# Copojacaab/APDA-FFT

Hardware: NVIDIA B200
Metric: FFT+peak windows/sec at N=4096 (higher is better)
Workload: dtype f32

## Files before the change

### apda-fft_b200/csrc/fft_f32_fast.cuh

```cuda
#pragma once
#include "common.cuh"

namespace {

__device__ __forceinline__ unsigned long long &u64(float2 &v) { return reinterpret_cast<unsigned long long &>(v); }
__device__ __forceinline__ const unsigned long long &u64(const float2 &v) {
    return reinterpret_cast<const unsigned long long &>(v);
}
__device__ __forceinline__ float2 cadd(float2 a, float2 b) {
    float2 r;
    asm("add.rn.f32x2 %0, %1, %2;" : "=l"(u64(r)) : "l"(u64(a)), "l"(u64(b)));
    return r;
}
__device__ __forceinline__ float2 csub(float2 a, float2 b) {
    float2 r;
    asm("sub.rn.f32x2 %0, %1, %2;" : "=l"(u64(r)) : "l"(u64(a)), "l"(u64(b)));
    return r;
}
__device__ __forceinline__ float2 pmul(float2 a, float2 b) {
    float2 r;
    asm("mul.rn.f32x2 %0, %1, %2;" : "=l"(u64(r)) : "l"(u64(a)), "l"(u64(b)));
    return r;
}
__device__ __forceinline__ float2 pfma(float2 a, float2 b, float2 c) {
    float2 r;
    asm("fma.rn.f32x2 %0, %1, %2, %3;" : "=l"(u64(r)) : "l"(u64(a)), "l"(u64(b)), "l"(u64(c)));
    return r;
}
__device__ __forceinline__ float2 cmul(float2 a, float2 w) {
    return make_float2(fmaf(a.x, w.x, -a.y * w.y), fmaf(a.x, w.y, a.y * w.x));
}

#define SQRT1_2f 0.70710678118654752440f
#define COS_PI_8f 0.92387953251128675613f
#define SIN_PI_8f 0.38268343236508977173f

__device__ __forceinline__ void add_sub_mi(float2 u, float2 d, float2 &plus, float2 &minus) {
    plus = make_float2(u.x + d.y, u.y - d.x);
    minus = make_float2(u.x - d.y, u.y + d.x);
}

__device__ __forceinline__ void fft4(float2 &a0, float2 &a1, float2 &a2, float2 &a3) {
    const float2 t0 = cadd(a0, a2), t1 = csub(a0, a2), t2 = cadd(a1, a3), d = csub(a1, a3);
    a0 = cadd(t0, t2);
    a2 = csub(t0, t2);
    add_sub_mi(t1, d, a1, a3);
}
__device__ __forceinline__ void fft8(float2 *v) {
    float2 e0 = v[0], e1 = v[2], e2 = v[4], e3 = v[6];
    float2 o0 = v[1], o1 = v[3], o2 = v[5], o3 = v[7];
    fft4(e0, e1, e2, e3);
    fft4(o0, o1, o2, o3);
    o1 = pmul(make_float2(o1.x + o1.y, o1.y - o1.x), make_float2(SQRT1_2f, SQRT1_2f));
    o3 = pmul(make_float2(o3.y - o3.x, o3.x + o3.y), make_float2(SQRT1_2f, -SQRT1_2f));
    v[0] = cadd(e0, o0);
    v[4] = csub(e0, o0);
    v[1] = cadd(e1, o1);
    v[5] = csub(e1, o1);
    add_sub_mi(e2, o2, v[2], v[6]);
    v[3] = cadd(e3, o3);
    v[7] = csub(e3, o3);
}
__device__ __forceinline__ void fft16(float2 *v) {
    float2 e[8], o[8];
#pragma unroll
    for (int i = 0; i < 8; ++i) {
        e[i] = v[2 * i];
        o[i] = v[2 * i + 1];
    }
    fft8(e);
    fft8(o);
    const float2 w1 = make_float2(COS_PI_8f, -SIN_PI_8f), w3 = make_float2(SIN_PI_8f, -COS_PI_8f);
    const float2 w5 = make_float2(-SIN_PI_8f, -COS_PI_8f), w7 = make_float2(-COS_PI_8f, -SIN_PI_8f);
    o[1] = cmul(o[1], w1);
    o[2] = pmul(make_float2(o[2].x + o[2].y, o[2].y - o[2].x), make_float2(SQRT1_2f, SQRT1_2f));
    o[3] = cmul(o[3], w3);
    o[5] = cmul(o[5], w5);
    o[6] = pmul(make_float2(o[6].y - o[6].x, o[6].x + o[6].y), make_float2(SQRT1_2f, -SQRT1_2f));
    o[7] = cmul(o[7], w7);
#pragma unroll
    for (int i = 0; i < 8; ++i) {
        if (i == 4) {
            add_sub_mi(e[4], o[4], v[4], v[12]);
        } else {
            v[i] = cadd(e[i], o[i]);
            v[i + 8] = csub(e[i], o[i]);
        }
    }
}
template <int R>
__device__ __forceinline__ void fft_r(float2 *v) {
    if (R == 16) fft16(v);
    else if (R == 8) fft8(v);
    else fft4(v[0], v[1], v[2], v[3]);
}

__constant__ float2 c_tw2_1024[64];
__constant__ float2 c_tw2_2048[64];
__constant__ float2 c_tw2_4096[128];
__constant__ float2 c_tw2_8192[256];
template <int N>
__device__ __forceinline__ const float2 *const_tw2() {
    return N == 1024 ? c_tw2_1024 : N == 2048 ? c_tw2_2048 : N == 4096 ? c_tw2_4096 : c_tw2_8192;
}

#ifndef APDA_K1_MINB_2048
#define APDA_K1_MINB_2048 8
#endif
#ifndef APDA_K1_MINB_1024
#define APDA_K1_MINB_1024 8
#endif
#ifndef APDA_K1_MINB_8192
#define APDA_K1_MINB_8192 4
#endif
#ifndef APDA_K1_MINB
#define APDA_K1_MINB 9
#endif
template <int N>
struct Plan;
template <>
struct Plan<8192> { static constexpr int R1 = 16, R2 = 16, R3 = 16, WPB = 1, MINB = APDA_K1_MINB_8192; };
template <>
struct Plan<4096> { static constexpr int R1 = 16, R2 = 16, R3 = 8, WPB = 1, MINB = APDA_K1_MINB; };
template <>
struct Plan<2048> { static constexpr int R1 = 16, R2 = 8, R3 = 8, WPB = 2, MINB = APDA_K1_MINB_2048; };
template <>
struct Plan<1024> { static constexpr int R1 = 8, R2 = 8, R3 = 8, WPB = 4, MINB = APDA_K1_MINB_1024; };

template <int T>
__device__ __forceinline__ void group_sync(int slot) {
    if (T == 32) __syncwarp();
    else if (slot == 0) asm volatile("bar.sync 1, %0;" ::"n"(T) : "memory");
    else asm volatile("bar.sync 2, %0;" ::"n"(T) : "memory");
}

__device__ __forceinline__ float next_above(float v) {
    float n = key_value(ordered_key(v) + 1u, 0.f);
    if (!(n > v)) n = key_value(ordered_key(v) + 2u, 0.f);
    return n;
}

__device__ __noinline__ float2 bracket_minmax(float2 a0, float2 a1, float2 a2, float2 a3, float2 a4, float2 a5, float2 a6,
                                              float2 a7, float2 a8, float2 a9, float2 a10, float2 a11, float2 a12, float2 a13,
                                              float2 a14, float2 a15, unsigned inb) {
    const float2 a[16] = {a0, a1, a2, a3, a4, a5, a6, a7, a8, a9, a10, a11, a12, a13, a14, a15};
    float vmin = CUDART_INF_F, vmax = -CUDART_INF_F;
#pragma unroll
    for (int i = 0; i < 16; ++i) {
        if (inb & (0x80000000u >> (2 * i))) {
            vmin = fminf(vmin, a[i].x);
            vmax = fmaxf(vmax, a[i].x);
        }
        if (inb & (0x80000000u >> (2 * i + 1))) {
            vmin = fminf(vmin, a[i].y);
            vmax = fmaxf(vmax, a[i].y);
        }
    }
#pragma unroll
    for (int o = 16; o > 0; o >>= 1) {
        vmin = fminf(vmin, __shfl_xor_sync(0xffffffffu, vmin, o));
        vmax = fmaxf(vmax, __shfl_xor_sync(0xffffffffu, vmax, o));
    }
    return make_float2(vmin, vmax);
}

constexpr int kTightenFrom = 4;
template <int T, bool FULL, typename Reload>
__device__ float select_median(const float2 (&v2)[16], int n_valid, uint32_t *sh , int t, int slot,
                               Reload reload ) {
#define VAL(i) (((i) & 1) ? v2[(i) >> 1].y : v2[(i) >> 1].x)
    constexpr int NW = (T + 31) / 32;
    const int lane = t & 31, warp = t >> 5;
    const int r_lo = (n_valid - 1) >> 1, r_hi = n_valid >> 1;
    float *shf = reinterpret_cast<float *>(sh);

    {
        float s1 = 0.f, s2 = 0.f;
        int cntv = 0;
#pragma unroll
        for (int c = 0; c < 16; c += 4) {
#pragma unroll
            for (int h = 0; h < 2; ++h) {
                const float raw = h ? v2[c].y : v2[c].x;
                const bool ok = FULL || raw < CUDART_INF_F;
                const float x = ok ? raw : 0.f;
                s1 += x;
                s2 = fmaf(x, x, s2);
                cntv += ok;
            }
        }
#pragma unroll
        for (int o = 16; o > 0; o >>= 1) {
            s1 += __shfl_xor_sync(0xffffffffu, s1, o);
            s2 += __shfl_xor_sync(0xffffffffu, s2, o);
        }
        if (!FULL) cntv = __reduce_add_sync(0xffffffffu, cntv);
        if (lane == 0) {
            shf[warp] = s1;
            shf[8 + warp] = s2;
            if (!FULL) sh[16 + warp] = (uint32_t)cntv;
        }
        if (t == 0) sh[48] = 0;
    }
    group_sync<T>(slot);
    float mean, sd;
    {
        float s1 = 0.f, s2 = 0.f;
        int cntv = FULL ? 8 * T : 0;
#pragma unroll
        for (int w = 0; w < NW; ++w) {
            s1 += shf[w];
            s2 += shf[8 + w];
            if (!FULL) cntv += (int)sh[16 + w];
        }
        const float inv = rcp_approx((float)max(cntv, 1));
        mean = s1 * inv;
        sd = sqrt_approx(fmaxf(fmaf(-mean, mean, s2 * inv), 0.f));
    }
    const float inv_density = fmaxf(2.5f * sd, 1e-30f) * rcp_approx((float)n_valid);

    float lo = -CUDART_INF_F, hi = CUDART_INF_F;
    int c_lo = 0, c_hi = n_valid;
    unsigned mask_lo = 0u, mask_hi = 0xffffffffu;
    if (!FULL) {
        mask_hi = 0u;
#pragma unroll
        for (int i = 0; i < 32; ++i) mask_hi = (mask_hi << 1) | (VAL(i) < CUDART_INF_F ? 1u : 0u);
    }
    float pivot = mean;
    for (int round = 0;; ++round) {
        if (round > 0) {
            if (c_hi - c_lo <= 32) break;
            if (round >= kTightenFrom) {
                const float2 mm = bracket_minmax(v2[0], v2[1], v2[2], v2[3], v2[4], v2[5], v2[6], v2[7], v2[8], v2[9], v2[10],
                                                 v2[11], v2[12], v2[13], v2[14], v2[15], ~mask_lo & mask_hi);
                if (lane == 0) {
                    shf[warp] = mm.x;
                    shf[8 + warp] = mm.y;
                }
                group_sync<T>(slot);
                float vmin = shf[0], vmax = shf[8];
#pragma unroll
                for (int w = 1; w < NW; ++w) {
                    vmin = fminf(vmin, shf[w]);
                    vmax = fmaxf(vmax, shf[8 + w]);
                }
                if (vmin == vmax) {
                    group_sync<T>(slot);
                    return vmin;
                }
                lo = vmin;
                hi = next_above(vmax);
            }
            const float lo_next = lo > -CUDART_INF_F ? next_above(lo) : -3.4028234e38f;
            if (!(lo_next < hi)) break;
            const float want = (float)r_lo + 0.5f;
            if (lo == -CUDART_INF_F) {
                pivot = hi - 1.5f * fmaxf((float)c_hi - want, 1.f) * inv_density * (float)(1 << min(round - 1, 20));
            } else if (hi == CUDART_INF_F) {
                pivot = lo + 1.5f * fmaxf(want - (float)c_lo, 1.f) * inv_density * (float)(1 << min(round - 1, 20));
            } else if (round % 3 == 2) {
                const uint32_t a = ordered_key(lo), b = ordered_key(hi);
                pivot = key_value(a + ((b - a) >> 1), 0.f);
            } else {
                pivot = lo + (hi - lo) * __fdividef(want - (float)c_lo, (float)(c_hi - c_lo));
            }
            if (!(pivot > lo)) pivot = lo_next;
            if (!(pivot < hi)) pivot = lo_next;
        }
        unsigned signs = 0;
        const float2 pv = make_float2(pivot, pivot);
#pragma unroll
        for (int i = 0; i < 16; ++i) {
            const float2 d = csub(v2[i], pv);
            signs = __funnelshift_l(__float_as_uint(d.x), signs, 1);
            signs = __funnelshift_l(__float_as_uint(d.y), signs, 1);
        }
        int cnt = __popc(signs);
        cnt = __reduce_add_sync(0xffffffffu, cnt);
        uint32_t *cslot = sh + 32 + 8 * (round & 1);
        if (lane == 0) cslot[warp] = (uint32_t)cnt;
        group_sync<T>(slot);
        int tot = 0;
#pragma unroll
        for (int w = 0; w < NW; ++w) tot += (int)cslot[w];
        if (tot <= r_lo) {
            lo = pivot;
            c_lo = tot;
            mask_lo = signs;
        } else if (tot > r_hi) {
            hi = pivot;
            c_hi = tot;
            mask_hi = signs;
        } else {
            float below = -CUDART_INF_F, above = CUDART_INF_F;
#pragma unroll
            for (int i = 0; i < 32; ++i) {
                if (VAL(i) < pivot) below = fmaxf(below, VAL(i));
                else above = fminf(above, VAL(i));
            }
#pragma unroll
            for (int o = 16; o > 0; o >>= 1) {
                below = fmaxf(below, __shfl_xor_sync(0xffffffffu, below, o));
                above = fminf(above, __shfl_xor_sync(0xffffffffu, above, o));
            }
            if (lane == 0) {
                shf[warp] = below;
                shf[8 + warp] = above;
            }
            group_sync<T>(slot);
#pragma unroll
            for (int w = 0; w < NW; ++w) {
                below = fmaxf(below, shf[w]);
                above = fminf(above, shf[8 + w]);
            }
            group_sync<T>(slot);
            return (below + above) * 0.5f;
        }
    }
    if (c_hi - c_lo > 32) {
        group_sync<T>(slot);
        return lo;
    }
    for (unsigned inb = ~mask_lo & mask_hi; inb; ) {
        const int q = __clz(inb);
        inb &= ~(0x80000000u >> q);
        const uint32_t pos = atomicAdd(&sh[48], 1u);
        if (pos < 32u) shf[pos] = reload(q);
    }
    group_sync<T>(slot);
    const int cnt = (int)sh[48];
    if (warp == 0) {
        float med;
        if (cnt > 32) {
            med = lo;
        } else {
            const float mine = lane < cnt ? shf[lane] : CUDART_INF_F;
            int rank = 0;
            for (int j = 0; j < cnt; ++j) {
                const float other = shf[j];
                rank += (other < mine) || (other == mine && j < lane);
            }
            const uint32_t m_lo = __ballot_sync(0xffffffffu, lane < cnt && rank == r_lo - c_lo);
            const uint32_t m_hi = __ballot_sync(0xffffffffu, lane < cnt && rank == r_hi - c_lo);
            const float a = __shfl_sync(0xffffffffu, mine, __ffs(m_lo) - 1);
            const float b = __shfl_sync(0xffffffffu, mine, __ffs(m_hi) - 1);
            med = (a + b) * 0.5f;
        }
        if (lane == 0) shf[49] = med;
    }
    group_sync<T>(slot);
    return shf[49];
}
#undef VAL

template <int N, int CENTER, bool FULL, int PF_AHEAD = 0>
__device__ __forceinline__ void k1_forward(const float *__restrict__ samples, const int n_samples, const int64_t ld,
                                           const int64_t winc, const float2 *__restrict__ tw1, float2 *s, uint32_t *sel_w,
                                           float *red_w, const int wslot, const int t, const int64_t pf_batch = 0) {
    constexpr int center = CENTER;
    using P = Plan<N>;
    constexpr int M = N / 2, R1 = P::R1, R2 = P::R2, R3 = P::R3, T = M / 16;
    constexpr int S1 = R2 * R3;
    constexpr int LD = S1 + 16 / R1;
    constexpr int G1 = 16 / R1, G2 = 16 / R2, G3 = 16 / R3;
    float2 v[16];
    const float *x = samples + winc * ld;
    const float2 *z = reinterpret_cast<const float2 *>(x);
    const bool full = FULL;
#pragma unroll
    for (int g = 0; g < G1; ++g) {
        const int c = t + T * g;
#pragma unroll
        for (int n1 = 0; n1 < R1; ++n1) {
            const int zi = n1 * S1 + c;
            float2 val;
            if (FULL) {
                val = __ldg(z + zi);
            } else {
                val.x = (2 * zi < n_samples) ? __ldg(x + 2 * zi) : 0.f;
                val.y = (2 * zi + 1 < n_samples) ? __ldg(x + 2 * zi + 1) : 0.f;
            }
            v[g * R1 + n1] = val;
        }
    }
    if (APDA_L2_PREFETCH && PF_AHEAD > 0) {
        const int64_t wn = winc + (int64_t)sm_count_reg() * PF_AHEAD;
        if (wn < pf_batch) l2_prefetch_span(samples + wn * ld, n_samples * (int)sizeof(float), t, T);
    }
    float shift = 0.f;
    if (center == APDA_CENTER_MEDIAN) {
        if (!full) {
#pragma unroll
            for (int g = 0; g < G1; ++g)
#pragma unroll
                for (int n1 = 0; n1 < R1; ++n1) {
                    const int zi = n1 * S1 + t + T * g;
                    if (2 * zi >= n_samples) v[g * R1 + n1].x = CUDART_INF_F;
                    if (2 * zi + 1 >= n_samples) v[g * R1 + n1].y = CUDART_INF_F;
                }
        }
        auto reload = [&](int q) {
            const int j = q >> 1;
            return __ldg(x + 2 * ((j % R1) * S1 + t + T * (j / R1)) + (q & 1));
        };
        shift = select_median<T, FULL>(v, n_samples, sel_w, t, wslot, reload);
        if (!full) {
#pragma unroll
            for (int i = 0; i < 16; ++i) {
                if (v[i].x == CUDART_INF_F) v[i].x = 0.f;
                if (v[i].y == CUDART_INF_F) v[i].y = 0.f;
            }
        }
    } else if (center == APDA_CENTER_MEAN) {
        float acc = 0.f;
#pragma unroll
        for (int i = 0; i < 16; ++i) acc += v[i].x + v[i].y;
#pragma unroll
        for (int o = 16; o > 0; o >>= 1) acc += __shfl_xor_sync(0xffffffffu, acc, o);
        if ((t & 31) == 0) red_w[t >> 5] = acc;
        group_sync<T>(wslot);
        float tot = 0.f;
#pragma unroll
        for (int w = 0; w < (T + 31) / 32; ++w) tot += red_w[w];
        shift = tot / (float)n_samples;
    }
#pragma unroll
    for (int g = 0; g < G1; ++g) {
        const int c = t + T * g;
        if (center != APDA_CENTER_NONE) {
#pragma unroll
            for (int n1 = 0; n1 < R1; ++n1) {
                const int zi = n1 * S1 + c;
                if (full) {
                    v[g * R1 + n1] = csub(v[g * R1 + n1], make_float2(shift, shift));
                } else {
                    if (2 * zi < n_samples) v[g * R1 + n1].x -= shift;
                    if (2 * zi + 1 < n_samples) v[g * R1 + n1].y -= shift;
                }
            }
        }
        fft_r<R1>(v + g * R1);
        s[c] = v[g * R1];
#pragma unroll
        for (int k1 = 1; k1 < R1; ++k1) s[k1 * LD + c] = cmul(v[g * R1 + k1], __ldg(tw1 + k1 * S1 + c));
    }
    group_sync<T>(wslot);

    const float2 *tw2 = const_tw2<N>();
#pragma unroll
    for (int g = 0; g < G2; ++g) {
        const int w = t + T * g;
        const int k1 = w % R1, n3 = w / R1;
        float2 *col = s + k1 * LD + n3;
#pragma unroll
        for (int n2 = 0; n2 < R2; ++n2) v[g * R2 + n2] = col[n2 * R3];
        fft_r<R2>(v + g * R2);
        col[0] = v[g * R2];
#pragma unroll
        for (int k2 = 1; k2 < R2; ++k2) col[k2 * R3] = cmul(v[g * R2 + k2], tw2[k2 * R3 + n3]);
    }
    group_sync<T>(wslot);

#pragma unroll
    for (int g = 0; g < G3; ++g) {
        const int w = t + T * g;
        const int k1 = w % R1, k2 = w / R1;
        const float2 *row = s + k1 * LD + k2 * R3;
#pragma unroll
        for (int n3 = 0; n3 < R3; ++n3) v[g * R3 + n3] = row[n3];
        fft_r<R3>(v + g * R3);
    }
    group_sync<T>(wslot);
#pragma unroll
    for (int g = 0; g < G3; ++g) {
        const int w = t + T * g;
#pragma unroll
        for (int k3 = 0; k3 < R3; ++k3) s[w + R1 * R2 * k3] = v[g * R3 + k3];
    }
    group_sync<T>(wslot);

}

}
```

Before: 80.57 million.

## Use two-pivot bracketing and sampled stats in median selection

Reworks the block-wide median selection used for centering. The mean and standard deviation now come from a per-warp sample of 256 input values, which removes a block synchronisation. Each round tests two pivots bracketing the target rank instead of one, so fewer rounds and fewer barriers should be needed. The final candidates are compacted deterministically with prefix sums instead of shared atomics, and every warp ranks them through shuffles. The costs are an approximate starting estimate, extra compare and popcount work per round, and more complex index bookkeeping.

```diff
diff --git a/apda-fft_b200/csrc/fft_f32_fast.cuh b/apda-fft_b200/csrc/fft_f32_fast.cuh
--- a/apda-fft_b200/csrc/fft_f32_fast.cuh
+++ b/apda-fft_b200/csrc/fft_f32_fast.cuh
@@ -164,29 +164,48 @@
     return make_float2(vmin, vmax);
 }
 
+__device__ __forceinline__ unsigned below_bits(const float2 (&v2)[16], float p) {
+    unsigned signs = 0;
+    const float2 pv = make_float2(p, p);
+#pragma unroll
+    for (int i = 0; i < 16; ++i) {
+        const float2 d = csub(v2[i], pv);
+        signs = __funnelshift_l(__float_as_uint(d.x), signs, 1);
+        signs = __funnelshift_l(__float_as_uint(d.y), signs, 1);
+    }
+    return signs;
+}
+
 constexpr int kTightenFrom = 4;
-template <int T, bool FULL, typename Reload>
-__device__ float select_median(const float2 (&v2)[16], int n_valid, uint32_t *sh , int t, int slot,
-                               Reload reload ) {
+constexpr float kFirstHalfWidth = 0.16f;
+constexpr int kGuardRanks = 13;
+template <int T, bool FULL>
+__device__ float select_median(const float2 (&v2)[16], int n_valid, const float *__restrict__ x ,
+                               uint32_t *sh , int t, int slot) {
 #define VAL(i) (((i) & 1) ? v2[(i) >> 1].y : v2[(i) >> 1].x)
     constexpr int NW = (T + 31) / 32;
+    static_assert(NW <= 8, "a bank holds 2 x 8 per-warp counts");
     const int lane = t & 31, warp = t >> 5;
     const int r_lo = (n_valid - 1) >> 1, r_hi = n_valid >> 1;
     float *shf = reinterpret_cast<float *>(sh);
 
+    float mean, sd;
     {
         float s1 = 0.f, s2 = 0.f;
-        int cntv = 0;
-#pragma unroll
-        for (int c = 0; c < 16; c += 4) {
-#pragma unroll
-            for (int h = 0; h < 2; ++h) {
-                const float raw = h ? v2[c].y : v2[c].x;
-                const bool ok = FULL || raw < CUDART_INF_F;
-                const float x = ok ? raw : 0.f;
-                s1 += x;
-                s2 = fmaf(x, x, s2);
-                cntv += ok;
+        if (FULL) {
+            const float2 *z = reinterpret_cast<const float2 *>(x);
+#pragma unroll
+            for (int j = 0; j < 4; ++j) {
+                const float2 a = __ldg(z + (32 * j + lane) * (T / 8));
+                s1 += a.x + a.y;
+                s2 = fmaf(a.x, a.x, fmaf(a.y, a.y, s2));
+            }
+        } else {
+#pragma unroll 4
+            for (int j = 0; j < 8; ++j) {
+                const float a = __ldg(x + (((32 * j + lane) * n_valid) >> 8));
+                s1 += a;
+                s2 = fmaf(a, a, s2);
             }
         }
 #pragma unroll
@@ -194,28 +213,8 @@
             s1 += __shfl_xor_sync(0xffffffffu, s1, o);
             s2 += __shfl_xor_sync(0xffffffffu, s2, o);
         }
-        if (!FULL) cntv = __reduce_add_sync(0xffffffffu, cntv);
-        if (lane == 0) {
-            shf[warp] = s1;
-            shf[8 + warp] = s2;
-            if (!FULL) sh[16 + warp] = (uint32_t)cntv;
-        }
-        if (t == 0) sh[48] = 0;
-    }
-    group_sync<T>(slot);
-    float mean, sd;
-    {
-        float s1 = 0.f, s2 = 0.f;
-        int cntv = FULL ? 8 * T : 0;
-#pragma unroll
-        for (int w = 0; w < NW; ++w) {
-            s1 += shf[w];
-            s2 += shf[8 + w];
-            if (!FULL) cntv += (int)sh[16 + w];
-        }
-        const float inv = rcp_approx((float)max(cntv, 1));
-        mean = s1 * inv;
-        sd = sqrt_approx(fmaxf(fmaf(-mean, mean, s2 * inv), 0.f));
+        mean = s1 * (1.f / 256.f);
+        sd = sqrt_approx(fmaxf(fmaf(-mean, mean, s2 * (1.f / 256.f)), 0.f));
     }
     const float inv_density = fmaxf(2.5f * sd, 1e-30f) * rcp_approx((float)n_valid);
 
@@ -227,8 +226,17 @@
 #pragma unroll
         for (int i = 0; i < 32; ++i) mask_hi = (mask_hi << 1) | (VAL(i) < CUDART_INF_F ? 1u : 0u);
     }
-    float pivot = mean;
-    for (int round = 0;; ++round) {
+    int src_lo = -1, src_hi = 2;
+    float pa, pb;
+    {
+        float d = kFirstHalfWidth * sd;
+        if (!(fabsf(mean) < CUDART_INF_F)) mean = 0.f;
+        if (!(d < CUDART_INF_F)) d = 0.f;
+        pa = fmaxf(mean - d, -3.4028234e38f);
+        pb = fminf(mean + d, 3.4028234e38f);
+    }
+    int round = 0;
+    for (;; ++round) {
         if (round > 0) {
             if (c_hi - c_lo <= 32) break;
             if (round >= kTightenFrom) {
@@ -256,47 +264,67 @@
             if (!(lo_next < hi)) break;
             const float want = (float)r_lo + 0.5f;
             if (lo == -CUDART_INF_F) {
-                pivot = hi - 1.5f * fmaxf((float)c_hi - want, 1.f) * inv_density * (float)(1 << min(round - 1, 20));
+                pb = hi - 1.5f * fmaxf((float)c_hi - want, 1.f) * inv_density * (float)(1 << min(round - 1, 20));
             } else if (hi == CUDART_INF_F) {
-                pivot = lo + 1.5f * fmaxf(want - (float)c_lo, 1.f) * inv_density * (float)(1 << min(round - 1, 20));
-            } else if (round % 3 == 2) {
+                pb = lo + 1.5f * fmaxf(want - (float)c_lo, 1.f) * inv_density * (float)(1 << min(round - 1, 20));
+            } else if (round % 3 == 0) {
                 const uint32_t a = ordered_key(lo), b = ordered_key(hi);
-                pivot = key_value(a + ((b - a) >> 1), 0.f);
+                pb = key_value(a + ((b - a) >> 1), 0.f);
             } else {
-                pivot = lo + (hi - lo) * __fdividef(want - (float)c_lo, (float)(c_hi - c_lo));
-            }
-            if (!(pivot > lo)) pivot = lo_next;
-            if (!(pivot < hi)) pivot = lo_next;
-        }
-        unsigned signs = 0;
-        const float2 pv = make_float2(pivot, pivot);
-#pragma unroll
-        for (int i = 0; i < 16; ++i) {
-            const float2 d = csub(v2[i], pv);
-            signs = __funnelshift_l(__float_as_uint(d.x), signs, 1);
-            signs = __funnelshift_l(__float_as_uint(d.y), signs, 1);
-        }
-        int cnt = __popc(signs);
-        cnt = __reduce_add_sync(0xffffffffu, cnt);
-        uint32_t *cslot = sh + 32 + 8 * (round & 1);
-        if (lane == 0) cslot[warp] = (uint32_t)cnt;
+                const float span = hi - lo, inv = __fdividef(1.f, (float)(c_hi - c_lo));
+                pa = lo + span * (((float)(r_lo - kGuardRanks - c_lo) + 0.5f) * inv);
+                pb = lo + span * (((float)(r_hi + kGuardRanks - c_lo) + 0.5f) * inv);
+            }
+            if (!(pb > lo && pb < hi)) pb = lo_next;
+            if (!(pa > lo && pa < pb)) pa = pb;
+        }
+        const bool two = pa < pb;
+        const unsigned sa = below_bits(v2, pa);
+        const unsigned sb = two ? below_bits(v2, pb) : sa;
+        const int ca = __reduce_add_sync(0xffffffffu, __popc(sa));
+        const int cb = two ? __reduce_add_sync(0xffffffffu, __popc(sb)) : ca;
+        uint32_t *bank = sh + 32 + 16 * (round & 1);
+        if (lane == 0) {
+            bank[warp] = (uint32_t)ca;
+            bank[8 + warp] = (uint32_t)cb;
+        }
         group_sync<T>(slot);
-        int tot = 0;
-#pragma unroll
-        for (int w = 0; w < NW; ++w) tot += (int)cslot[w];
-        if (tot <= r_lo) {
-            lo = pivot;
-            c_lo = tot;
-            mask_lo = signs;
-        } else if (tot > r_hi) {
-            hi = pivot;
-            c_hi = tot;
-            mask_hi = signs;
-        } else {
+        int ta = 0, tb = 0;
+#pragma unroll
+        for (int w = 0; w < NW; ++w) {
+            ta += (int)bank[w];
+            tb += (int)bank[8 + w];
+        }
+        if (src_lo >= 0) src_lo = 2;
+        src_hi = 2;
+        if (tb <= r_lo) {
+            lo = pb;
+            c_lo = tb;
+            mask_lo = sb;
+            src_lo = 1;
+        } else if (ta <= r_lo) {
+            lo = pa;
+            c_lo = ta;
+            mask_lo = sa;
+            src_lo = 0;
+        }
+        if (ta > r_hi) {
+            hi = pa;
+            c_hi = ta;
+            mask_hi = sa;
+            src_hi = 0;
+        } else if (tb > r_hi) {
+            hi = pb;
+            c_hi = tb;
+            mask_hi = sb;
+            src_hi = 1;
+        }
+        if (c_hi - c_lo > 32 && ((ta > r_lo && ta <= r_hi) || (tb > r_lo && tb <= r_hi))) {
+            const float pivot = (ta > r_lo && ta <= r_hi) ? pa : pb;
             float below = -CUDART_INF_F, above = CUDART_INF_F;
 #pragma unroll
             for (int i = 0; i < 32; ++i) {
-                if (VAL(i) < pivot) below = fmaxf(below, VAL(i));
+                if (__float_as_uint(VAL(i) - pivot) >> 31) below = fmaxf(below, VAL(i));
                 else above = fminf(above, VAL(i));
             }
 #pragma unroll
@@ -322,35 +350,54 @@
         group_sync<T>(slot);
         return lo;
     }
-    for (unsigned inb = ~mask_lo & mask_hi; inb; ) {
-        const int q = __clz(inb);
-        inb &= ~(0x80000000u >> q);
-        const uint32_t pos = atomicAdd(&sh[48], 1u);
-        if (pos < 32u) shf[pos] = reload(q);
+    const unsigned inb = ~mask_lo & mask_hi;
+    const int cnt = c_hi - c_lo;
+    int pos = 0;
+    if (NW > 1) {
+        if (src_lo < 2 && src_hi < 2) {
+            const uint32_t *last = sh + 32 + 16 * ((round - 1) & 1);
+#pragma unroll
+            for (int w = 0; w < NW; ++w)
+                if (w < warp) pos += (int)last[8 * src_hi + w] - (src_lo < 0 ? 0 : (int)last[8 * src_lo + w]);
+        } else {
+            uint32_t *other = sh + 32 + 16 * (round & 1);
+            const int mine = __reduce_add_sync(0xffffffffu, __popc(inb));
+            if (lane == 0) other[warp] = (uint32_t)mine;
+            group_sync<T>(slot);
+#pragma unroll
+            for (int w = 0; w < NW; ++w)
+                if (w < warp) pos += (int)other[w];
+        }
+    }
+    {
+        const int own = __popc(inb);
+        int incl = own;
+#pragma unroll
+        for (int o = 1; o < 32; o <<= 1) {
+            const int y = __shfl_up_sync(0xffffffffu, incl, o);
+            if (lane >= o) incl += y;
+        }
+        pos += incl - own;
+    }
+    if (inb) {
+#pragma unroll
+        for (int q = 0; q < 32; ++q) {
+            if (inb & (0x80000000u >> q)) shf[pos++] = VAL(q);
+        }
     }
     group_sync<T>(slot);
-    const int cnt = (int)sh[48];
-    if (warp == 0) {
-        float med;
-        if (cnt > 32) {
-            med = lo;
-        } else {
-            const float mine = lane < cnt ? shf[lane] : CUDART_INF_F;
-            int rank = 0;
-            for (int j = 0; j < cnt; ++j) {
-                const float other = shf[j];
-                rank += (other < mine) || (other == mine && j < lane);
-            }
-            const uint32_t m_lo = __ballot_sync(0xffffffffu, lane < cnt && rank == r_lo - c_lo);
-            const uint32_t m_hi = __ballot_sync(0xffffffffu, lane < cnt && rank == r_hi - c_lo);
-            const float a = __shfl_sync(0xffffffffu, mine, __ffs(m_lo) - 1);
-            const float b = __shfl_sync(0xffffffffu, mine, __ffs(m_hi) - 1);
-            med = (a + b) * 0.5f;
-        }
-        if (lane == 0) shf[49] = med;
-    }
-    group_sync<T>(slot);
-    return shf[49];
+    const float mine = lane < cnt ? shf[lane] : CUDART_INF_F;
+    int rank = 0;
+    for (int j = 0; j < cnt; ++j) {
+        const float other = __shfl_sync(0xffffffffu, mine, j);
+        rank += (other < mine) || (other == mine && j < lane);
+    }
+    const uint32_t m_lo = __ballot_sync(0xffffffffu, lane < cnt && rank == r_lo - c_lo);
+    const float a = __shfl_sync(0xffffffffu, mine, __ffs(m_lo) - 1);
+    if (r_lo == r_hi) return a;
+    const uint32_t m_hi = __ballot_sync(0xffffffffu, lane < cnt && rank == r_hi - c_lo);
+    const float b = __shfl_sync(0xffffffffu, mine, __ffs(m_hi) - 1);
+    return (a + b) * 0.5f;
 }
 #undef VAL
 
@@ -400,11 +447,7 @@
                     if (2 * zi + 1 >= n_samples) v[g * R1 + n1].y = CUDART_INF_F;
                 }
         }
-        auto reload = [&](int q) {
-            const int j = q >> 1;
-            return __ldg(x + 2 * ((j % R1) * S1 + t + T * (j / R1)) + (q & 1));
-        };
-        shift = select_median<T, FULL>(v, n_samples, sel_w, t, wslot, reload);
+        shift = select_median<T, FULL>(v, n_samples, x, sel_w, t, wslot);
         if (!full) {
 #pragma unroll
             for (int i = 0; i < 16; ++i) {
```

After: 68.88 million, median of 6. 14.5% lower.
